# BICLab/Spike2Former

Measured on AMD Instinct MI355X. Metric: fwd+bwd images/sec, 512x512 T=4 ADE20K-150, higher is better.
Workload: dtype f32 (fp32-equivalent: bf16 hi+mid+lo split operands on bf16 MFMA, fp32 accumulate; spike maps stored as bf16, exact); 1 GPU; C2: 512x512 T=4 K=150 Meta-SpikeFormer [64, 128, 256, 360] + MaskFormer head, per-GPU batch 2; global_batch=2, parallelism=dp1, weights=random-init (name-seeded)

## Files before the change

include/s2f.h:

```cpp
#ifndef S2F_H
#define S2F_H

#include <stdint.h>

#ifdef __cplusplus
extern "C" {
#endif

#define S2F_OK 0
#define S2F_EINVAL (-1)
#define S2F_EALIGN (-2)
#define S2F_ELAUNCH (-3)

#define S2F_ABI_VERSION 36
#define S2F_STAT_SLOTS 256

int s2f_version(void);
const char* s2f_last_error(void);

void* s2f_event_create(void);
void s2f_event_destroy(void* event);
int s2f_time_next_call(void* start_event, void* stop_event);
int s2f_event_elapsed_us(void* start_event, void* stop_event, double* microseconds);

int64_t s2f_lif_mask_words(int64_t n);

int s2f_lif_fwd(const float* x, const float* v_in, void* y, float* v_out, uint64_t* mask, uint8_t* count_u8,
                uint64_t* stats, int64_t n, float vth, int D, int y_bf16, void* stream);

int s2f_lif_bwd(const float* gy, const float* gv_out, const uint64_t* mask, float* gx, int64_t n, float vth, int D,
                void* stream);
int s2f_lif_bwd_ports(const float* gy, const float* gy2, const float* gv_out, const uint64_t* mask, const float* skip, float* gx,
                      int64_t n, float vth, int D, void* stream);

int s2f_lif_leaky_fwd(const float* x, const float* v_in, void* y, float* v_out, uint64_t* mask, uint64_t* stats, int64_t n, float vth,
                      int D, float tau, int decay_input, int y_bf16, void* stream);
int s2f_lif_leaky_bwd(const float* gy, const float* gv_out, const uint64_t* mask, float* gx, float* gv_in, int64_t n, float vth, int D,
// ... 94 lines not shown
int s2f_spike_gemm_dw_pipe_ok(int batch, int M, int K, int L);
int s2f_spike_gemm_dw_pipe(const float* dY, const uint16_t* X, float* dW, int batch, int M, int K, int L, int accumulate, int cfg,
                           int target_wgs, void* stream);
int s2f_spike_gemm_dw_pipe_grouped(const int64_t* jobs, int njobs, int cfg, int target_wgs, void* stream);
int s2f_spike_conv3x3_dw_pipe_ok(int batch, int M, int C, int H, int W);
int s2f_shift1_bf16(const uint16_t* X, uint16_t* Xs, int64_t n, void* stream);
int s2f_spike_conv3x3_dw_pipe(const int64_t* jobs, int njobs, int cfg, int target_wgs, void* stream);

int s2f_gemm_bn_lif_fwd(const uint16_t* a_pack, const uint16_t* X, const float* conv_bias, const float* running_mean,
                        const float* running_var, const float* gamma, const float* beta, float eps, const float* residual,
                        float* u_out, const float* v_in, void* y_bf16, float* v_out, uint64_t* stats, int batch, int M, int N,
                        int K, float vth, int D, void* stream);
int s2f_conv3x3_bn_lif_fwd(const uint16_t* w_pack, const uint16_t* X, const float* conv_bias, const float* running_mean,
                           const float* running_var, const float* gamma, const float* beta, float eps, const float* residual,
                           float* u_out, const float* v_in, void* y_bf16, float* v_out, uint64_t* stats, int batch, int M, int C,
                           int H, int W, float vth, int D, void* stream);
int64_t s2f_pack_elems(int M, int K);
int s2f_pack_bf16x3(const float* src, uint16_t* dst, int M, int K, int mode, int C, void* stream);
int s2f_pack_bf16x3_multi(const int64_t* jobs, int njobs, int64_t total_workgroups, void* stream);
int s2f_pgemm_nn_bf16(const uint16_t* a_pack, const uint16_t* X, const float* bias, float* Y, int batch, int M, int N, int K,
                      int terms, int cfg, void* stream);
int s2f_pgemm_dx_f32(const uint16_t* w_pack, const float* G, int64_t g_batch_stride, float* DX, int64_t dx_batch_stride,
                     int batch, int Mo, int Ki, int N, float beta, int cfg, void* stream);
int s2f_dense_gemm_bn_lif_fwd(const uint16_t* const* w_packs, int groups, const float* X, int64_t x_batch_stride, int64_t x_group_stride,
                              const float* conv_bias, const float* running_mean, const float* running_var, const float* gamma,
                              const float* beta, float eps, const float* residual, float* u_out, void* y_bf16, uint64_t* stats,
                              int batch, int K, int M, int N, float vth, int D, void* stream);
int s2f_pgemm_dx_f32_grouped(const uint16_t* const* w_packs, int groups, const float* G, int64_t g_batch_stride,
                             int64_t g_group_stride, float* DX, int64_t dx_batch_stride, int64_t dx_group_stride, float* bn_partials,
                             int64_t partials_group_stride, int batch, int Mo, int Ki, int N, void* stream);
int s2f_pgemm_conv3x3_bf16(const uint16_t* w_pack, const uint16_t* X, const float* bias, float* Y, int batch, int M, int C, int H,
                           int W, int cfg, void* stream);
int s2f_pgemm_conv3x3_f32(const uint16_t* w_pack, const float* X, float* Y, int batch, int M, int C, int H, int W, int cfg,
                          void* stream);
int64_t s2f_bn_partials_count(int batch, int N);
int s2f_pgemm_nn_bf16_stats(const uint16_t* a_pack, const uint16_t* X, float* Y, float* bn_partials, int batch, int M, int N, int K,
                            void* stream);
int s2f_pgemm_conv3x3_bf16_stats(const uint16_t* w_pack, const uint16_t* X, float* Y, float* bn_partials, int batch, int M, int C,
                                 int H, int W, void* stream);
int s2f_pgemm_dx_f32_stats(const uint16_t* w_pack, const float* G, int64_t g_batch_stride, float* DX, int64_t dx_batch_stride,
                           float* bn_partials, int batch, int Mo, int Ki, int N, void* stream);
int s2f_bn_partials_finalize(const float* partials, int64_t P, const float* conv_bias, double* sums_out, int64_t N, int64_t C,
                             int64_t L, void* stream);
int s2f_bn_bwd_ports_ok(int64_t N, int64_t C, int64_t L, int training, int D);
int s2f_bn_act_bwd_ports(const float* z, const float* conv_bias, const float* stat, const float* gamma, const float* g_u,
                         const float* g_y, const float* g_y2, const float* g_v, const uint64_t* mask, double* sums_zeroed, float* gz,
// ... 136 lines not shown
```

spike2former_amd/_lib.py:

```python
import ctypes
import os

import torch

_HERE = os.path.dirname(os.path.abspath(__file__))
LIB_PATH = os.environ.get("S2F_LIB") or os.path.join(_HERE, "libs2f_hip.so")

_p, _i, _i64, _f = ctypes.c_void_p, ctypes.c_int, ctypes.c_int64, ctypes.c_float

SIGNATURES = {
    "s2f_version": (_i, []),
    "s2f_last_error": (ctypes.c_char_p, []),
    "s2f_event_create": (_p, []),
    "s2f_event_destroy": (None, [_p]),
    "s2f_time_next_call": (_i, [_p, _p]),
    "s2f_event_elapsed_us": (_i, [_p, _p, ctypes.POINTER(ctypes.c_double)]),
    "s2f_lif_mask_words": (_i64, [_i64]),
    "s2f_lif_fwd": (_i, [_p, _p, _p, _p, _p, _p, _p, _i64, _f, _i, _i, _p]),
    "s2f_lif_bwd": (_i, [_p, _p, _p, _p, _i64, _f, _i, _p]),
    "s2f_lif_bwd_ports": (_i, [_p] * 6 + [_i64, _f, _i, _p]),
    "s2f_lif_leaky_fwd": (_i, [_p, _p, _p, _p, _p, _p, _i64, _f, _i, _f, _i, _i, _p]),
    "s2f_lif_leaky_bwd": (_i, [_p, _p, _p, _p, _p, _i64, _f, _i, _f, _i, _p]),
    "s2f_sum2_lif_fwd": (_i, [_p] * 7 + [_i64] * 4 + [_f, _i, _i, _p]),
    "s2f_sum2_lif_bwd": (_i, [_p] * 5 + [_i64, _i, _p]),
# ... 43 lines not shown
    "s2f_split_gemm": (_i, [_p, _i64, _i64, _i, _p, _i64, _i, _i64, _i, _p, _i64, _f, _i, _i, _i, _i, _i, _i, _p]),
    "s2f_spike_gemm_dw": (_i, [_p, _p, _p, _i, _i, _i, _i, _i, _i, _p]),
    "s2f_to_bf16_exact": (_i, [_p, _p, _i64, _p]),
    "s2f_spike_gemm_fwd_bf16": (_i, [_p] * 4 + [_i] * 7 + [_p]),
    "s2f_spike_conv3x3_fwd_bf16": (_i, [_p, _p, _p, _p] + [_i] * 8 + [_p]),
    "s2f_spike_gemm_dw_bf16": (_i, [_p, _p, _p, _i, _i, _i, _i, _i, _p]),
    "s2f_spike_gemm_fwd_bf16_ex": (_i, [_p, _i64, _p, _i64, _i, _i64, _p, _i64, _f, _p, _i, _i, _i, _i, _i, _i, _p]),
    "s2f_pgemm_nn_bf16_ex": (_i, [_p, _i64, _p, _i64, _i, _i64, _p, _i64, _f, _p, _i, _i, _i, _i, _p]),
    "s2f_spike_gemm_dw_grouped": (_i, [_p, _i, _i, _p]),
    "s2f_spike_gemm_dw_pipe_ok": (_i, [_i] * 4),
    "s2f_spike_gemm_dw_pipe": (_i, [_p, _p, _p] + [_i] * 7 + [_p]),
    "s2f_spike_gemm_dw_pipe_grouped": (_i, [_p, _i, _i, _i, _p]),
    "s2f_spike_conv3x3_dw_pipe_ok": (_i, [_i] * 5),
    "s2f_shift1_bf16": (_i, [_p, _p, _i64, _p]),
    "s2f_spike_conv3x3_dw_pipe": (_i, [_p, _i, _i, _i, _p]),
    "s2f_spike_conv3x3_dw_bf16": (_i, [_p, _p, _p] + [_i] * 6 + [_p]),
    "s2f_gemm_bn_lif_fwd": (_i, [_p] * 7 + [_f] + [_p] * 6 + [_i] * 4 + [_f, _i, _p]),
    "s2f_conv3x3_bn_lif_fwd": (_i, [_p] * 7 + [_f] + [_p] * 6 + [_i] * 5 + [_f, _i, _p]),
    "s2f_pack_elems": (_i64, [_i, _i]),
    "s2f_pack_bf16x3_multi": (_i, [_p, _i, _i64, _p]),
    "s2f_pgemm_nn_bf16": (_i, [_p] * 4 + [_i] * 6 + [_p]),
    "s2f_pack_bf16x3": (_i, [_p, _p, _i, _i, _i, _i, _p]),
    "s2f_pgemm_dx_f32": (_i, [_p, _p, _i64, _p, _i64] + [_i] * 4 + [_f, _i, _p]),
    "s2f_gemm_dw_general": (_i, [_p, _i64, _p, _i64, _p] + [_i] * 5 + [_p]),
    "s2f_pgemm_conv3x3_bf16": (_i, [_p, _p, _p, _p] + [_i] * 6 + [_p]),
    "s2f_pgemm_conv3x3_f32": (_i, [_p, _p, _p] + [_i] * 6 + [_p]),
    "s2f_gemm_dw_general_grouped": (_i, [_p, _i, _p]),
    "s2f_bn_partials_count": (_i64, [_i, _i]),
    "s2f_pgemm_nn_bf16_stats": (_i, [_p] * 4 + [_i] * 4 + [_p]),
    "s2f_pgemm_conv3x3_bf16_stats": (_i, [_p] * 4 + [_i] * 5 + [_p]),
    "s2f_pgemm_dx_f32_grouped": (_i, [_p, _i, _p, _i64, _i64, _p, _i64, _i64, _p, _i64] + [_i] * 4 + [_p]),
    "s2f_dense_gemm_bn_lif_fwd": (_i, [_p, _i, _p, _i64, _i64, _p, _p, _p, _p, _p, _f, _p, _p, _p, _p, _i, _i, _i, _i, _f, _i, _p]),
    "s2f_pgemm_dx_f32_stats": (_i, [_p, _p, _i64, _p, _i64, _p] + [_i] * 4 + [_p]),
    "s2f_bn_partials_finalize": (_i, [_p, _i64, _p, _p, _i64, _i64, _i64, _p]),
    "s2f_bn_act_bwd_split": (_i, [_p] * 13 + [_i64] * 3 + [_i, _f, _i, _p]),
    "s2f_bn_act_bwd_ports": (_i, [_p] * 14 + [_i64] * 3 + [_i, _f, _i, _p]),
    "s2f_bn_bwd_ports_ok": (_i, [_i64, _i64, _i64, _i, _i]),
    "s2f_mask_cost_bins": (_i, [_p, _p, _p, _i, _i, _i64, _i, _f, _f, _f, _p]),
    "s2f_mask_loss_seg_partials": (_i64, [_i] * 4),
    "s2f_mask_loss_seg_fwd": (_i, [_p] * 5 + [_i] * 4 + [_f, _f, _p]),
    "s2f_mask_loss_seg_bwd": (_i, [_p] * 5 + [_i] * 4 + [_f, _f, _p]),
    "s2f_lsa_tables": (_i, [_p] * 6 + [_i] * 4 + [_p]),
    "s2f_lsa_tables_ex": (_i, [_p] * 6 + [_i] * 5 + [_p]),
    "s2f_spike_gemm_dw_bf16_split": (_i, [_p, _i64, _p, _p] + [_i] * 5 + [_p]),
    "s2f_spike_gemm_dw_grouped_split": (_i, [_p, _i, _i, _p]),
    "s2f_pgemm_dx_split": (_i, [_p, _p, _i64, _p] + [_i] * 5 + [_p]),
# ... 54 lines not shown
```

spike2former_amd/csrc/pgemm.hip:

```cpp
#include "gemm_common.h"
#include <cstdlib>
#include <type_traits>

#pragma clang fp contract(fast)

namespace {

constexpr int PK = 32;
constexpr int PR = 64;
constexpr int PTERM = PR * PK;
constexpr int PBLOCK = 3 * PTERM;

typedef __attribute__((address_space(3))) void lds_void;
typedef const __attribute__((address_space(1))) void gbl_void;

__device__ __forceinline__ void dma16(const void* src, void* lds_dst) {
  __builtin_amdgcn_global_load_lds((gbl_void*)src, (lds_void*)lds_dst, 16, 0, 0);
}
template <int OFF>
__device__ __forceinline__ s16x4 lds_tr16_asm(unsigned byte_addr) {
  s16x4 r;
  asm volatile("ds_read_b64_tr_b16 %0, %1 offset:%2" : "=v"(r) : "v"(byte_addr), "n"(OFF));
  return r;
}
// ... 397 lines not shown
      const int row = m0 + wm * (32 * MI) + i * 32 + (r & 3) + 8 * (r >> 2) + 4 * (lane >> 5);
      bv[r] = bias ? bias[min(row, M - 1)] : 0.f;
    }
#pragma unroll
    for (int j = 0; j < NJ; ++j) {
      const int col = n0 + (wn * NJ + j) * 32 + (lane & 31);
#pragma unroll
      for (int r = 0; r < 16; ++r) {
        const int row = m0 + wm * (32 * MI) + i * 32 + (r & 3) + 8 * (r >> 2) + 4 * (lane >> 5);
        if (row < M && col < N) Yb[(int64_t)row * N + col] = EX ? (acc[i][j][r] + bv[r]) * ex.out_scale : acc[i][j][r] + bv[r];
      }
    }
  }
  if constexpr (STATS)
    epi_row_partials<MI, NJ, WMW, WNW>(acc, part, n_tiles * (int)gridDim.y, reinterpret_cast<float*>(smem), m0, n0, M, N,
                                       b * n_tiles + nt, wm, wn, lane, (int)threadIdx.x);
}

struct TnGroups {
  const unsigned short* wp[4];
  int64_t g_stride, dx_stride, part_stride;
};

template <int MI, int NJ, int WMW, int WNW, int EPI, int KS = 1, bool STATS = false, bool GROUPED = false>
__global__ __launch_bounds__(64 * WMW * WNW) void pg_tn_f32_kernel(const unsigned short* __restrict__ Wp,
                                                                  const float* __restrict__ G, float* __restrict__ DX, int Mo,
                                                                  int Ki, int N, int KbW, int n_tiles, int m_tiles, float beta,
                                                                  int64_t g_batch_stride, int64_t dx_batch_stride,
                                                                  float* __restrict__ part = nullptr, TnGroups grp = TnGroups{},
                                                                  BnLifEpi ep = BnLifEpi{}) {
  if constexpr (GROUPED) {
    static_assert(EPI == 0 || EPI == 3, "grouped form: plain store or the eval-mode BatchNorm epilogue");
    const int g = blockIdx.z;
    Wp = grp.wp[g];
    G += g * grp.g_stride;
    if (EPI == 0) DX += g * grp.dx_stride;
    if (STATS) part += g * grp.part_stride;
    if constexpr (EPI == 3) {
      if (ep.conv_bias) ep.conv_bias += g * Ki;
      ep.mean += g * Ki, ep.var += g * Ki, ep.gamma += g * Ki, ep.beta += g * Ki;
      if (ep.residual) ep.residual += g * grp.dx_stride;
      if (ep.u_out) ep.u_out += g * grp.dx_stride;
      if (ep.y) ep.y += g * grp.dx_stride;
    }
  }
  constexpr bool BETA = EPI == 1;
  constexpr int BM = 32 * MI * WMW, BN = 32 * NJ * WNW, NW = WMW * WNW, T = 64 * NW;
  constexpr int KC = 16 * KS;
  constexpr int A_SLICE = 3 * (BM / 32) * 1024;
  constexpr int A_BYTES = KS * A_SLICE, B_TERM = KC * BN * 2, B_BYTES = 3 * B_TERM, STAGE = A_BYTES + B_BYTES;
  constexpr int NA = 3 * (BM / 32);
  constexpr int NQ = KC * BN / 4 / T;
  static_assert(NQ >= 1 && (KC * BN / 4) % T == 0, "tile too small for the thread count");
  __shared__ __attribute__((aligned(1024))) unsigned char smem[2 * STAGE];

  const int tiles = n_tiles * m_tiles;
  int pid = blockIdx.x;
  if (tiles % 8 == 0) pid = (pid % 8) * (tiles / 8) + pid / 8;
  const int mt = pid % m_tiles, nt = pid / m_tiles;
  const int b = blockIdx.y;
  const int m0 = mt * BM, n0 = nt * BN;
  const float* Gb = G + (int64_t)b * g_batch_stride;
  float* Db = DX + (int64_t)b * dx_batch_stride;
  const int tid = threadIdx.x, lane = tid & 63;
  const int wave = __builtin_amdgcn_readfirstlane((int)(tid >> 6));
  const int wm = wave / WNW, wn = wave % WNW;
  const int nk_all = (Mo + KC - 1) / KC;
  const int per_z = (nk_all + (int)gridDim.z - 1) / (int)gridDim.z;
  const int t_first = EPI == 2 ? (int)blockIdx.z * per_z : 0;
  const int nk = EPI == 2 ? max(0, min(nk_all - t_first, per_z)) : nk_all;
  if (EPI == 2 && nk == 0) return;

  auto issue_a = [&](int tl, int st) __attribute__((always_inline)) {
    unsigned char* sb = smem + st * STAGE;
#pragma unroll
    for (int ks = 0; ks < KS; ++ks) {
      const int c0 = (t_first + tl) * KC + 16 * ks;
      const unsigned short* rows = Wp + (int64_t)(c0 / PR) * KbW * PBLOCK + (c0 % PR) * PK + lane * 8;
#pragma unroll
      for (int q = 0; q < (NA + NW - 1) / NW; ++q) {
        const int idx = wave + q * NW;
        if (NA % NW != 0 && idx >= NA) break;
        const int term = idx / (BM / 32), p = idx % (BM / 32);
        const int kb = min(m0 / PK + p, KbW - 1);
// ... 20 lines not shown
      const int k = p / (BN / 4), c4 = p % (BN / 4);
      const int off = k * BN + ((((c4 >> 3) ^ (k & 3)) << 5) | ((c4 & 7) << 2));
      unsigned int h0, m0_, l0_, h1, m1, l1;
      s2f_split3x2(breg[q].x, breg[q].y, h0, m0_, l0_);
      s2f_split3x2(breg[q].z, breg[q].w, h1, m1, l1);
      *reinterpret_cast<u32x2*>(Bs + off) = u32x2{h0, h1};
      *reinterpret_cast<u32x2*>(Bs + KC * BN + off) = u32x2{m0_, m1};
      *reinterpret_cast<u32x2*>(Bs + 2 * KC * BN + off) = u32x2{l0_, l1};
    }
  };

  f32x16 acc[MI][NJ];
#pragma unroll
  for (int i = 0; i < MI; ++i)
#pragma unroll
    for (int j = 0; j < NJ; ++j)
#pragma unroll
      for (int r = 0; r < 16; ++r) acc[i][j][r] = 0.f;

  const int kl = (lane & 15) >> 2, piece = lane & 3, hcol = (lane >> 4) & 1, kh = lane >> 5;
  int boff[NJ];
#pragma unroll
  for (int j = 0; j < NJ; ++j) boff[j] = (8 * kh + kl) * BN + (((wn * NJ + j) ^ kl) << 5) + 16 * hcol + 4 * piece;
  int aoff[MI][2];
#pragma unroll
  for (int i = 0; i < MI; ++i)
#pragma unroll
    for (int half = 0; half < 2; ++half) {
      const int row = 8 * kh + kl + 4 * half;
      const int c = (2 * hcol + (piece >> 1)) ^ ((2 * kh + half) & 3);
      aoff[i][half] = (wm * MI + i) * 512 + row * 32 + c * 8 + 4 * (piece & 1);
    }

  const unsigned smem_a = lds_addr(smem);
  auto compute = [&](int st) __attribute__((always_inline)) {
    union BF {
      bf16x8 v;
      s16x4 h[2];
    } bfrag[3][NJ], afrag[3][MI];
    const unsigned sb0 = smem_a + st * STAGE;
#pragma unroll
    for (int ks = 0; ks < KS; ++ks) {
      const unsigned sb = sb0 + ks * A_SLICE;
      const unsigned sbb = sb0 + ks * (16 * BN * 2);
#pragma unroll
      for (int j = 0; j < NJ; ++j) {
        const unsigned a = sbb + boff[j] * 2;
        bfrag[0][j].h[0] = lds_tr16_asm<A_BYTES>(a);
        bfrag[0][j].h[1] = lds_tr16_asm<A_BYTES + 4 * BN * 2>(a);
        bfrag[1][j].h[0] = lds_tr16_asm<A_BYTES + B_TERM>(a);
        bfrag[1][j].h[1] = lds_tr16_asm<A_BYTES + B_TERM + 4 * BN * 2>(a);
        bfrag[2][j].h[0] = lds_tr16_asm<A_BYTES + 2 * B_TERM>(a);
        bfrag[2][j].h[1] = lds_tr16_asm<A_BYTES + 2 * B_TERM + 4 * BN * 2>(a);
      }
#pragma unroll
      for (int i = 0; i < MI; ++i) {
        afrag[0][i].h[0] = lds_tr16_asm<0>(sb + aoff[i][0] * 2);
        afrag[0][i].h[1] = lds_tr16_asm<0>(sb + aoff[i][1] * 2);
      }
#pragma unroll
      for (int i = 0; i < MI; ++i) {
        afrag[1][i].h[0] = lds_tr16_asm<(BM / 32) * 1024>(sb + aoff[i][0] * 2);
        afrag[1][i].h[1] = lds_tr16_asm<(BM / 32) * 1024>(sb + aoff[i][1] * 2);
      }
#pragma unroll
      for (int i = 0; i < MI; ++i) {
        afrag[2][i].h[0] = lds_tr16_asm<2 * (BM / 32) * 1024>(sb + aoff[i][0] * 2);
        afrag[2][i].h[1] = lds_tr16_asm<2 * (BM / 32) * 1024>(sb + aoff[i][1] * 2);
      }
#pragma unroll
      for (int ta = 0; ta < 3; ++ta) {
        if (ta == 0) lds_wait<4 * MI>();
        if (ta == 1) lds_wait<2 * MI>();
        if (ta == 2) lds_wait<0>();
#pragma unroll
        for (int i = 0; i < MI; ++i)
#pragma unroll
          for (int tb = 0; tb < 3; ++tb)
            if (ta + tb < 3)
#pragma unroll
              for (int j = 0; j < NJ; ++j)
                mfma_bf16(acc[i][j], afrag[ta][i].v, bfrag[tb][j].v);
      }
    }
  };

  fetch_b(0);
  issue_a(0, 0);
  stage_b(0);
  if (nk > 1) fetch_b(1);
  for (int t = 0; t < nk; ++t) {
    const int st = t & 1;
    if (t + 1 < nk)
      wait_vm_and_barrier<NQ>();
    else
      wait_vm_and_barrier<0>();
    if (t + 1 < nk) {
      stage_b(st ^ 1);
      issue_a(t + 1, st ^ 1);
      if (t + 2 < nk) fetch_b(t + 2);
    }
    compute(st);
  }

  mfma_fence(acc);
  if constexpr (EPI == 3) {
    static_assert(2 * STAGE >= BM * BN * 4, "the output tile must fit the stages it is transposed through");
    epi_bn_lif<MI, NJ, WMW, WNW>(acc, ep, smem, m0, n0, Ki, N, b, wm, wn, lane, wave, dx_batch_stride);
    return;
  }
#pragma unroll
  for (int i = 0; i < MI; ++i)
#pragma unroll
    for (int j = 0; j < NJ; ++j) {
      const int col = n0 + (wn * NJ + j) * 32 + (lane & 31);
      float prev[16];
      if (BETA) {
#pragma unroll
        for (int r = 0; r < 16; ++r) {
          const int row = m0 + (wm * MI + i) * 32 + (r & 3) + 8 * (r >> 2) + 4 * (lane >> 5);
          prev[r] = Db[(int64_t)min(row, Ki - 1) * N + min(col, N - 1)];
        }
      }
#pragma unroll
      for (int r = 0; r < 16; ++r) {
        const int row = m0 + (wm * MI + i) * 32 + (r & 3) + 8 * (r >> 2) + 4 * (lane >> 5);
        if (row < Ki && col < N) {
          if (EPI == 2)
            atomicAdd(Db + (int64_t)row * N + col, acc[i][j][r]);
          else
            Db[(int64_t)row * N + col] = BETA ? acc[i][j][r] + beta * prev[r] : acc[i][j][r];
        }
      }
    }
  if constexpr (EPI == 0 && STATS)
    epi_row_partials<MI, NJ, WMW, WNW>(acc, part, n_tiles * (int)gridDim.y, reinterpret_cast<float*>(smem), m0, n0, Ki, N,
                                       b * n_tiles + nt, wm, wn, lane, tid);
}

template <int MI, int NJ, int WMW, int WNW, int NST>
__global__ __launch_bounds__(64 * WMW * WNW) void pg_tn_split_kernel(const unsigned short* __restrict__ Wp,
                                                                    const unsigned short* __restrict__ Gs, int64_t plane_stride,
                                                                    float* __restrict__ DX, int Mo, int Ki, int N, int KbW,
                                                                    int n_tiles, int m_tiles) {
  constexpr int BM = 32 * MI * WMW, BN = 32 * NJ * WNW, NW = WMW * WNW;
  constexpr int KC = 16;
  constexpr int A_BYTES = 3 * (BM / 32) * 1024, B_TERM = KC * BN * 2, B_BYTES = 3 * B_TERM, STAGE = A_BYTES + B_BYTES;
  constexpr int NA = 3 * (BM / 32), NAW = (NA + NW - 1) / NW;
  constexpr int NBT = B_TERM / 1024, NB = 3 * NBT, NBW = NB / NW;
  static_assert(NB % NW == 0 && BN == 128, "tile shape");
  constexpr int LPW = NAW + NBW;
  __shared__ __attribute__((aligned(1024))) unsigned char smem[NST * STAGE];

  const int tiles = n_tiles * m_tiles;
  int pid = blockIdx.x;
  if (tiles % 8 == 0) pid = (pid % 8) * (tiles / 8) + pid / 8;
  const int mt = pid % m_tiles, nt = pid / m_tiles;
// ... 460 lines not shown
constexpr bool conv_g2_built(int cfg) {
  for (const ConvForm& f : kConvForms)
    if (f.g == 2 && (f.cfgs >> cfg & 1)) return true;
  return false;
}

constexpr PgTile kTnSplitTiles[] = {
    {1, 2, 2, 2, 2, 3},
    {2, 1, 2, 2, 2, 3},
    {3, 2, 2, 2, 2, 2},
    {4, 1, 2, 2, 2, 2},
};

constexpr PgTile kTnTiles[] = {
    {1, 2, 2, 2, 2, 1},
    {2, 1, 2, 2, 2, 1},
    {3, 1, 2, 4, 2, 1},
    {4, 1, 1, 2, 4, 1},
    {5, 1, 1, 1, 4, 1},
    {7, 1, 1, 2, 4, 2},
    {8, 1, 2, 2, 2, 2},
    {9, 1, 2, 4, 2, 2},
    {10, 1, 1, 2, 4, 4},
};
struct TnForm {
  int epi;
  bool stats, grouped;
  unsigned cfgs;
};
constexpr TnForm kTnForms[] = {
    {2, false, false, cfg_set(1, 2, 3, 4, 5)},
    {1, false, false, cfg_set(1, 2, 3, 4, 5)},
    {0, true, false, cfg_set(1, 2, 3, 4, 5, 7, 8, 9, 10)},
    {0, false, false, cfg_set(1, 2, 3, 4, 5, 7, 8, 9, 10)},
    {0, true, true, cfg_set(3, 5, 7)},
    {0, false, true, cfg_set(3, 5, 7)},
    {3, false, true, cfg_set(5, 7, 9, 10)},
};

bool launch_pg_nn(int cfg, int terms, int epi, bool ex_form, hipStream_t s, const uint16_t* a_pack, const uint16_t* X, const float* bias,
                  float* Y, int batch, int M, int N, int K, int64_t xbs, const BnLifEpi& ep, float* part, const NnEx& ex) {
  const int Kb = (K + PK - 1) / PK, n_tiles = (N + 127) / 128;
  bool ok = false;
  s2f_dispatch<kNnForms>(
      [&](const NnForm& e) { return e.terms == terms && e.epi == epi && e.stats == (part != nullptr) && e.ex == ex_form; }, [&](auto f) {
        constexpr NnForm F = kNnForms[f];
        ok = s2f_dispatch<kNnTiles>([&](const PgTile& e) { return e.cfg == cfg && (F.cfgs >> e.cfg & 1); }, [&](auto i) {
          constexpr PgTile T = kNnTiles[i];
          if constexpr (F.cfgs >> T.cfg & 1) {
            const int m_tiles = (M + T.rows() - 1) / T.rows();
            S2F_LAUNCH(true, true, (pg_nn_kernel<T.MI, T.NJ, T.WMW, T.WNW, F.terms, T.extra, F.epi, F.stats, F.ex>),
                       dim3(n_tiles * m_tiles, batch), dim3(T.threads()), 0, s, a_pack, X, bias, Y, M, N, K, Kb, n_tiles, m_tiles, xbs,
                       ep, part, ex);
          }
        });
      });
  return ok;
}

template <class TwoSteps>
bool launch_pg_conv(int cfg, bool conv, int bt, int epi, const TwoSteps& two_steps, hipStream_t s, const uint16_t* a_pack, const void* X,
                    const float* bias, float* Y, int batch, int M, int N, int K, int Kb, Conv3 geo, float* part, const BnLifEpi& ep) {
  const int n_tiles = (N + 127) / 128;
  bool ok = false;
  s2f_dispatch<kConvTiles>([&](const PgTile& e) { return e.cfg == cfg && (e.extra != 0) == conv; }, [&](auto i) {
    constexpr PgTile T = kConvTiles[i];
    const int m_tiles = (M + T.rows() - 1) / T.rows();
    const bool stats = part != nullptr && bt == 1;
    const int g = (conv_g2_built(T.cfg) && two_steps((int64_t)n_tiles * m_tiles * batch)) ? 2 : 1;
    ok = s2f_dispatch<kConvForms>(
        [&](const ConvForm& e) { return e.bt == bt && e.epi == epi && e.stats == stats && e.g == g && (e.cfgs >> T.cfg & 1); }, [&](auto f) {
          constexpr ConvForm F = kConvForms[f];
          if constexpr (F.cfgs >> T.cfg & 1)
            S2F_LAUNCH(true, true, (pg_conv_kernel<T.MI, T.NJ, T.WMW, T.WNW, F.bt, T.extra != 0, F.stats, F.epi, F.g>),
                       dim3(n_tiles * m_tiles, batch), dim3(T.threads()), 0, s, a_pack, X, bias, Y, M, N, K, Kb, n_tiles, m_tiles, geo,
                       part, ep);
        });
  });
  return ok;
}

bool launch_pg_tn(int cfg, int epi, bool grouped, hipStream_t s, const uint16_t* w_pack, const float* G, float* DX, int batch, int zdim,
                  int Mo, int Ki, int N, float beta, int64_t g_batch_stride, int64_t dx_batch_stride, float* part, const TnGroups& grp,
                  const BnLifEpi& ep) {
  const int KbW = (Ki + PK - 1) / PK, n_tiles = (N + 127) / 128;
  bool ok = false;
  s2f_dispatch<kTnForms>([&](const TnForm& e) { return e.epi == epi && e.stats == (part != nullptr) && e.grouped == grouped; }, [&](auto f) {
    constexpr TnForm F = kTnForms[f];
    ok = s2f_dispatch<kTnTiles>([&](const PgTile& e) { return e.cfg == cfg && (F.cfgs >> e.cfg & 1); }, [&](auto i) {
      constexpr PgTile T = kTnTiles[i];
      if constexpr (F.cfgs >> T.cfg & 1) {
        const int m_tiles = (Ki + T.rows() - 1) / T.rows();
        S2F_LAUNCH(true, true, (pg_tn_f32_kernel<T.MI, T.NJ, T.WMW, T.WNW, F.epi, T.extra, F.stats, F.grouped>),
                   dim3(n_tiles * m_tiles, batch, zdim), dim3(T.threads()), 0, s, w_pack, G, DX, Mo, Ki, N, KbW, n_tiles, m_tiles, beta,
                   g_batch_stride, dx_batch_stride, part, grp, ep);
      }
    });
  });
  return ok;
}

}

extern "C" int64_t s2f_pack_elems(int M, int K) { return (int64_t)((M + PR - 1) / PR) * ((K + PK - 1) / PK) * PBLOCK; }

extern "C" int s2f_pack_bf16x3_multi(const int64_t* jobs, int njobs, int64_t total_workgroups, void* stream) {
  if (njobs == 0) return S2F_OK;
  S2F_REQUIRE(jobs && njobs > 0 && total_workgroups > 0 && total_workgroups < (1ll << 31), S2F_EINVAL,
              "s2f_pack_bf16x3_multi: bad job table");
  hipLaunchKernelGGL(pack_multi_kernel, dim3((unsigned)total_workgroups), dim3(256), 0, (hipStream_t)stream,
                     reinterpret_cast<const long long*>(jobs), njobs);
  return s2f_check_launch("s2f_pack_bf16x3_multi");
}

static int pgemm_nn_impl(const uint16_t* a_pack, const uint16_t* X, const float* bias, float* Y, int batch, int M, int N, int K,
                         int terms, int cfg, float* part, void* stream) {
  S2F_REQUIRE(a_pack && X && Y, S2F_EINVAL, "s2f_pgemm_nn_bf16: null pointer");
  S2F_REQUIRE(!part || (!bias && (reinterpret_cast<uintptr_t>(part) & 7u) == 0), S2F_EINVAL,
// ... 153 lines not shown
  return conv_launch("s2f_pgemm_conv3x3_bf16", w_pack, X, false, bias, Y, batch, M, C, H, W, cfg, stream);
}

extern "C" int s2f_pgemm_conv3x3_bf16_stats(const uint16_t* w_pack, const uint16_t* X, float* Y, float* bn_partials, int batch,
                                            int M, int C, int H, int W, void* stream) {
  S2F_REQUIRE(bn_partials, S2F_EINVAL, "s2f_pgemm_conv3x3_bf16_stats: null partials");
  return conv_launch("s2f_pgemm_conv3x3_bf16_stats", w_pack, X, false, nullptr, Y, batch, M, C, H, W, 0, stream, bn_partials);
}

extern "C" int s2f_pgemm_conv3x3_f32(const uint16_t* w_pack, const float* X, float* Y, int batch, int M, int C, int H, int W,
                                     int cfg, void* stream) {
  return conv_launch("s2f_pgemm_conv3x3_f32", w_pack, X, true, nullptr, Y, batch, M, C, H, W, cfg, stream);
}

extern "C" int s2f_pack_bf16x3(const float* src, uint16_t* dst, int M, int K, int mode, int C, void* stream) {
  S2F_REQUIRE(src && dst && M > 0 && K > 0 && mode >= 0 && mode <= 3, S2F_EINVAL, "s2f_pack_bf16x3: bad arguments");
  S2F_REQUIRE((mode != 1 && mode != 2) || C > 0, S2F_EINVAL, "s2f_pack_bf16x3: conv modes need C");
  const int64_t wgs = (int64_t)((M + PR - 1) / PR) * ((K + PK - 1) / PK) * (PTERM / 1024);
  hipLaunchKernelGGL(pack_one_kernel, dim3((unsigned)wgs), dim3(256), 0, (hipStream_t)stream, src, dst, M, K, mode, C);
  return s2f_check_launch("s2f_pack_bf16x3");
}

static int pgemm_dx_impl(const uint16_t* w_pack, const float* G, int64_t g_batch_stride, float* DX, int64_t dx_batch_stride,
                         int batch, int Mo, int Ki, int N, float beta, int cfg, float* part, void* stream) {
  if (g_batch_stride == 0) g_batch_stride = (int64_t)Mo * N;
  S2F_REQUIRE(!part || (beta == 0.f && (reinterpret_cast<uintptr_t>(part) & 7u) == 0), S2F_EINVAL,
              "s2f_pgemm_dx_f32_stats: plain-store form only; partials 8-byte aligned");
  if (dx_batch_stride == 0) dx_batch_stride = (int64_t)Ki * N;
  S2F_REQUIRE((g_batch_stride & 3) == 0 && (dx_batch_stride & 3) == 0, S2F_EALIGN, "s2f_pgemm_dx_f32: batch strides must keep 16-byte alignment");
  S2F_REQUIRE(w_pack && G && DX, S2F_EINVAL, "s2f_pgemm_dx_f32: null pointer");
  S2F_REQUIRE(batch > 0 && batch < 65536 && Mo > 0 && Ki > 0 && N >= 4 && (N & 3) == 0, S2F_EINVAL,
              "s2f_pgemm_dx_f32: bad sizes (N=%d must be a positive multiple of 4)", N);
  S2F_REQUIRE(s2f_aligned16(w_pack) && s2f_aligned16(G) && s2f_aligned16(DX), S2F_EALIGN,
              "s2f_pgemm_dx_f32: pointers must be 16-byte aligned");
  hipStream_t s = (hipStream_t)stream;
  const int n_tiles = (N + 127) / 128;
  static const char* force = getenv("S2F_PG_DX_CFG");
  int c = cfg > 0 ? cfg : (force ? atoi(force) : 0);
  static const char* t3e = getenv("S2F_PG_DX_T3");
  const int64_t t3 = t3e ? atoll(t3e) : 192;
  if (c <= 0) c = Ki <= 32 ? 5 : (Ki > 64 && (int64_t)n_tiles * batch * ((Ki + 127) / 128) >= t3) ? 3 : (beta == 0.f ? 7 : 4);
  static const char* ks4 = getenv("S2F_PG_DX_KS4");
  if (c == 7 && !(ks4 && ks4[0] == '0') && Mo >= 128 && (int64_t)n_tiles * batch * ((Ki + 63) / 64) <= 512) c = 10;
  int zsplit = 1;
  {
    const int64_t wgs = (int64_t)n_tiles * batch * ((Ki + 63) / 64);
    const int steps = (Mo + 15) / 16;
    while ((beta == 0.f || beta == 1.f) && !part && wgs * zsplit < 128 && steps / (zsplit * 2) >= 16) zsplit *= 2;
  }
  if (zsplit > 1) {
    S2F_REQUIRE(dx_batch_stride == (int64_t)Ki * N, S2F_EINVAL, "s2f_pgemm_dx_f32: the split form needs a dense DX");
    if (beta == 0.f && s2f_zero_async(DX, sizeof(float) * (size_t)batch * Ki * N, s) != S2F_OK)
      return s2f_check_launch("s2f_pgemm_dx_f32 zero");
    c = 4;
  }
  S2F_REQUIRE(c < 7 || c > 10 || (zsplit == 1 && beta == 0.f), S2F_EINVAL, "s2f_pgemm_dx_f32: cfg %d is the plain store form", c);
  const bool ok = launch_pg_tn(c, zsplit > 1 ? 2 : beta != 0.f ? 1 : 0, false, s, w_pack, G, DX, batch, zsplit, Mo, Ki, N, beta,
                               g_batch_stride, dx_batch_stride, part, TnGroups{}, BnLifEpi{});
  S2F_REQUIRE(ok, S2F_EINVAL, "s2f_pgemm_dx_f32: unknown cfg %d", c);
  return s2f_check_launch("s2f_pgemm_dx_f32");
}

extern "C" int s2f_pgemm_dx_f32(const uint16_t* w_pack, const float* G, int64_t g_batch_stride, float* DX,
                                int64_t dx_batch_stride, int batch, int Mo, int Ki, int N, float beta, int cfg, void* stream) {
  return pgemm_dx_impl(w_pack, G, g_batch_stride, DX, dx_batch_stride, batch, Mo, Ki, N, beta, cfg, nullptr, stream);
}

extern "C" int s2f_pgemm_dx_f32_stats(const uint16_t* w_pack, const float* G, int64_t g_batch_stride, float* DX,
                                      int64_t dx_batch_stride, float* bn_partials, int batch, int Mo, int Ki, int N,
                                      void* stream) {
  S2F_REQUIRE(bn_partials, S2F_EINVAL, "s2f_pgemm_dx_f32_stats: null partials");
  return pgemm_dx_impl(w_pack, G, g_batch_stride, DX, dx_batch_stride, batch, Mo, Ki, N, 0.f, 0, bn_partials, stream);
}

extern "C" int s2f_dense_gemm_bn_lif_fwd(const uint16_t* const* w_packs, int groups, const float* X, int64_t x_batch_stride,
                                         int64_t x_group_stride, const float* conv_bias, const float* running_mean,
                                         const float* running_var, const float* gamma, const float* beta, float eps,
                                         const float* residual, float* u_out, void* y_bf16, uint64_t* stats, int batch, int K,
                                         int M, int N, float vth, int D, void* stream) {
  S2F_REQUIRE(w_packs && X && running_mean && running_var && gamma && beta && groups >= 1 && groups <= 4, S2F_EINVAL,
              "s2f_dense_gemm_bn_lif_fwd: null pointer / 1..4 groups");
  S2F_REQUIRE(u_out || y_bf16, S2F_EINVAL, "s2f_dense_gemm_bn_lif_fwd: neither u_out nor y requested");
  S2F_REQUIRE(batch > 0 && batch < 65536 && M > 0 && K > 0 && N >= 4 && (N & 3) == 0, S2F_EINVAL,
// ... 51 lines not shown
```

spike2former_amd/ops/gemm.py:

```python
import torch

from .config import cfg
from .core import *
from .misc import channel_sum, transpose_last2




def bmm_small(a, b, reduce_batch=False):
    _need_cuda(a, b)
    B, M, K = a.shape
    N = b.shape[2]
    if b.shape[0] != B or b.shape[1] != K:
        raise RuntimeError(f"bmm_small: {tuple(a.shape)} @ {tuple(b.shape)}")
    c = torch.empty((M, N) if reduce_batch else (B, M, N), dtype=torch.float32, device=a.device)
    if c.numel() == 0:
        return c
    if K == 0 or B == 0:
        return c.zero_()
    check(lib.s2f_bmm_f32(_ptr(a), a.stride(0), a.stride(1), a.stride(2), _ptr(b), b.stride(0), b.stride(1), b.stride(2), _ptr(c),
                          0 if reduce_batch else M * N, N, 1, B, M, N, K, int(bool(reduce_batch)), _stream()), "s2f_bmm_f32")
    return c


# ... 615 lines not shown
                for t in range(T):
                    for b in range(B):
                        check(lib.s2f_spike_gemm_dw(_ptr(g[b]), _ptr(mf[t, b]), _ptr(ge[t, b]), 1, Q, C, HW, 1, 3, _stream()),
                              "s2f_spike_gemm_dw")
            else:
                ge = torch.stack([bmm_small(g, mf[t].transpose(1, 2)) for t in range(T)], 0)
            ge.mul_(ctx.scale)
        if ctx.needs_input_grad[1]:
            gmf = torch.empty_like(mf)
            if ctx.mfma:
                et = e.permute(0, 1, 3, 2).reshape(T * B * C, Q)
                a_split, Rpad, Kpad = _split_rows(et, 128)
                for t in range(T):
                    check(lib.s2f_split_gemm(_ptr(a_split) + 2 * t * B * C * Kpad, C * Kpad, Rpad * Kpad, 1, _ptr(g), Q * HW, Q,
                                             0, 3, _ptr(gmf[t]), C * HW, ctx.scale, B, C, HW, Q, (C + 127) // 128 * 128, Kpad,
                                             _stream()), "s2f_split_gemm")
            else:
                es = e * ctx.scale
                for t in range(T):
                    gmf[t].copy_(bmm_small(es[t].transpose(1, 2), g))
        return ge, gmf, None, None


def mask_einsum(e, mf, scale, e_exact=False):
    return _MaskEinsum.apply(e, mf, float(scale), bool(e_exact))


class _MaskEinsumFolded(torch.autograd.Function):

    @staticmethod
    def forward(ctx, e, sdata, stok, W, bias, scale, T, B, e_exact):
        _need_cuda(e, W, bias, spikes=sdata)
        Q, Co = e.shape[2], e.shape[3]
        C, HW = sdata.shape[1], sdata.shape[2]
        e = e.contiguous()
        sdata = sdata.contiguous()
        dev = e.device
        ew = _mm_tm(e.reshape(-1, Co), transpose_last2(W.detach().unsqueeze(0))[0]).view(T, B, Q, C)
        acat = ew.permute(1, 2, 0, 3).reshape(B, Q, T * C).contiguous()
        rowb = None
        if bias is not None:
            rowb = (e.sum(0) * bias.view(1, 1, -1)).sum(-1).contiguous()
        out = torch.empty(B, Q, HW, dtype=torch.float32, device=dev)
        if HW % 8 == 0 and C % 32 == 0:
            pe = int(lib.s2f_pack_elems(Q, T * C))
            a_pack = torch.empty(B, pe, dtype=torch.int16, device=dev)
# ... 7 lines not shown
            Kpad = T * C
            a_split = torch.empty(B, 3, Mpad, Kpad, dtype=torch.int16, device=dev)
            for b in range(B):
                check(lib.s2f_split_bf16x3(_ptr(acat[b]), _ptr(a_split[b]), Q, T * C, Mpad, Kpad, _stream()), "s2f_split_bf16x3")
            _time_next("spike_gemm_fwd", 4 * B * HW * (T * C + Q), 2 * B * Q * HW * T * C, moved=B * HW * (2 * T * C + 4 * Q))
            check(lib.s2f_spike_gemm_fwd_bf16_ex(_ptr(a_split), 3 * Mpad * Kpad, _ptr(sdata), C * HW, C, B * C * HW, _ptr(rowb),
                                                 Q if rowb is not None else 0, scale, _ptr(out), B, Q, HW, T * C, Mpad, Kpad, _stream()),
                  "s2f_spike_gemm_fwd_bf16_ex")
        ctx.save_for_backward(e, sdata, W, bias, ew)
        ctx.cfg = (scale, T, B)
        return out

    @staticmethod
    def backward(ctx, g):
        e, sdata, W, bias, ew = ctx.saved_tensors
        scale, T, B = ctx.cfg
        Q, Co = e.shape[2], e.shape[3]
        C, HW = sdata.shape[1], sdata.shape[2]
        g = g.contiguous()
        dev = g.device
        gs = ge = gW = gb = None
        S = sdata.view(T, B, C, HW)
        if (ctx.needs_input_grad[1] or ctx.needs_input_grad[2]) and HW % 4 == 0:
            ews = ew * scale
            gs = torch.empty(T * B, C, HW, dtype=torch.float32, device=dev)
            _time_next("dx_gemm", 4 * T * B * HW * (C + Q), 2 * T * B * Q * HW * C)
            for t in range(T):
                for b in range(B):
                    _mtm_tm(ews[t, b], g[b], out=gs[t * B + b])
        elif ctx.needs_input_grad[1] or ctx.needs_input_grad[2]:
            G = torch.empty(T, B, Co, HW, dtype=torch.float32, device=dev)
            es = e * scale
            for t in range(T):
                G[t].copy_(bmm_small(es[t].transpose(1, 2), g))
            gs = dx_gemm(W, G.view(T * B, Co, HW))
        if ctx.needs_input_grad[0] or ctx.needs_input_grad[3] or ctx.needs_input_grad[4]:
            H = torch.empty(T, B, Q, C, dtype=torch.float32, device=dev)
            xb = sdata.dtype == torch.bfloat16
            _time_next("spike_gemm_dw", 4 * T * B * HW * (C + Q), 2 * T * B * Q * HW * C, moved=T * B * HW * ((2 if xb else 4) * C + 4 * Q))
            if xb and T * B <= 56 and HW % 4 == 0:
                import ctypes
                H.zero_()
                flat = []
                for t in range(T):
                    for b in range(B):
                        flat += [g[b].data_ptr(), S[t, b].data_ptr(), H[t, b].data_ptr(), 1, Q, C, HW]
                arr = (ctypes.c_int64 * len(flat))(*flat)
                if (cfg.DW_PIPE and lib.s2f_spike_gemm_dw_pipe_ok(1, Q, C, HW) and g.data_ptr() % 16 == 0 and S.data_ptr() % 16 == 0
                        and (Q * HW) % 4 == 0 and (C * HW) % 8 == 0):
                    check(lib.s2f_spike_gemm_dw_pipe_grouped(arr, T * B, 0, 0, _stream()), "s2f_spike_gemm_dw_pipe_grouped")
                else:
                    check(lib.s2f_spike_gemm_dw_grouped(arr, T * B, 64, _stream()), "s2f_spike_gemm_dw_grouped")
# ... 46 lines not shown
```

Before: 56.41 images/s.

## Batch mask-einsum input gradient into one stacked row-block dx GEMM launch

```diff
diff --git a/include/s2f.h b/include/s2f.h
--- a/include/s2f.h
+++ b/include/s2f.h
@@ -12,7 +12,7 @@
 #define S2F_EALIGN (-2)
 #define S2F_ELAUNCH (-3)
 
-#define S2F_ABI_VERSION 36
+#define S2F_ABI_VERSION 37
 #define S2F_STAT_SLOTS 256
 
 int s2f_version(void);
@@ -153,6 +153,9 @@
                       int terms, int cfg, void* stream);
 int s2f_pgemm_dx_f32(const uint16_t* w_pack, const float* G, int64_t g_batch_stride, float* DX, int64_t dx_batch_stride,
                      int batch, int Mo, int Ki, int N, float beta, int cfg, void* stream);
+int s2f_pgemm_dx_f32_rowblocks(const uint16_t* w_pack, int64_t w_batch_stride, const float* G, int64_t g_batch_stride, float* DX,
+                               int64_t dx_batch_stride, int rows_per_block, int64_t block_stride, int batch, int Mo, int Ki, int N,
+                               int cfg, void* stream);
 int s2f_dense_gemm_bn_lif_fwd(const uint16_t* const* w_packs, int groups, const float* X, int64_t x_batch_stride, int64_t x_group_stride,
                               const float* conv_bias, const float* running_mean, const float* running_var, const float* gamma,
                               const float* beta, float eps, const float* residual, float* u_out, void* y_bf16, uint64_t* stats,
diff --git a/spike2former_amd/_lib.py b/spike2former_amd/_lib.py
--- a/spike2former_amd/_lib.py
+++ b/spike2former_amd/_lib.py
@@ -89,6 +89,7 @@
     "s2f_pgemm_nn_bf16": (_i, [_p] * 4 + [_i] * 6 + [_p]),
     "s2f_pack_bf16x3": (_i, [_p, _p, _i, _i, _i, _i, _p]),
     "s2f_pgemm_dx_f32": (_i, [_p, _p, _i64, _p, _i64] + [_i] * 4 + [_f, _i, _p]),
+    "s2f_pgemm_dx_f32_rowblocks": (_i, [_p, _i64, _p, _i64, _p, _i64, _i, _i64] + [_i] * 5 + [_p]),
     "s2f_gemm_dw_general": (_i, [_p, _i64, _p, _i64, _p] + [_i] * 5 + [_p]),
     "s2f_pgemm_conv3x3_bf16": (_i, [_p, _p, _p, _p] + [_i] * 6 + [_p]),
     "s2f_pgemm_conv3x3_f32": (_i, [_p, _p, _p] + [_i] * 6 + [_p]),
diff --git a/spike2former_amd/csrc/pgemm.hip b/spike2former_amd/csrc/pgemm.hip
--- a/spike2former_amd/csrc/pgemm.hip
+++ b/spike2former_amd/csrc/pgemm.hip
@@ -443,13 +443,15 @@
   int64_t g_stride, dx_stride, part_stride;
 };
 
-template <int MI, int NJ, int WMW, int WNW, int EPI, int KS = 1, bool STATS = false, bool GROUPED = false>
-__global__ __launch_bounds__(64 * WMW * WNW) void pg_tn_f32_kernel(const unsigned short* __restrict__ Wp,
+template <int MI, int NJ, int WMW, int WNW, int EPI, int KS = 1, bool STATS = false, bool GROUPED = false, bool ROWBLK = false>
+__global__ __launch_bounds__(64 * WMW * WNW, (MI * WMW == 8 ? 4 : 1)) void pg_tn_f32_kernel(const unsigned short* __restrict__ Wp,
                                                                   const float* __restrict__ G, float* __restrict__ DX, int Mo,
                                                                   int Ki, int N, int KbW, int n_tiles, int m_tiles, float beta,
                                                                   int64_t g_batch_stride, int64_t dx_batch_stride,
                                                                   float* __restrict__ part = nullptr, TnGroups grp = TnGroups{},
-                                                                  BnLifEpi ep = BnLifEpi{}) {
+                                                                  BnLifEpi ep = BnLifEpi{}, int rows_per_block = 0,
+                                                                  int64_t block_stride = 0, int64_t w_batch_stride = 0) {
+  static_assert(!ROWBLK || (EPI == 0 && !STATS && !GROUPED), "row blocks: the plain-store form only");
   if constexpr (GROUPED) {
     static_assert(EPI == 0 || EPI == 3, "grouped form: plain store or the eval-mode BatchNorm epilogue");
     const int g = blockIdx.z;
@@ -481,6 +483,7 @@
   const int mt = pid % m_tiles, nt = pid / m_tiles;
   const int b = blockIdx.y;
   const int m0 = mt * BM, n0 = nt * BN;
+  if constexpr (ROWBLK) Wp += (int64_t)b * w_batch_stride;
   const float* Gb = G + (int64_t)b * g_batch_stride;
   float* Db = DX + (int64_t)b * dx_batch_stride;
   const int tid = threadIdx.x, lane = tid & 63;
@@ -547,15 +550,13 @@
   int boff[NJ];
 #pragma unroll
   for (int j = 0; j < NJ; ++j) boff[j] = (8 * kh + kl) * BN + (((wn * NJ + j) ^ kl) << 5) + 16 * hcol + 4 * piece;
-  int aoff[MI][2];
-#pragma unroll
-  for (int i = 0; i < MI; ++i)
-#pragma unroll
-    for (int half = 0; half < 2; ++half) {
-      const int row = 8 * kh + kl + 4 * half;
-      const int c = (2 * hcol + (piece >> 1)) ^ ((2 * kh + half) & 3);
-      aoff[i][half] = (wm * MI + i) * 512 + row * 32 + c * 8 + 4 * (piece & 1);
-    }
+  int aoff[2];
+#pragma unroll
+  for (int half = 0; half < 2; ++half) {
+    const int row = 8 * kh + kl + 4 * half;
+    const int c = (2 * hcol + (piece >> 1)) ^ ((2 * kh + half) & 3);
+    aoff[half] = wm * MI * 512 + row * 32 + c * 8 + 4 * (piece & 1);
+  }
 
   const unsigned smem_a = lds_addr(smem);
   auto compute = [&](int st) __attribute__((always_inline)) {
@@ -578,20 +579,26 @@
         bfrag[2][j].h[0] = lds_tr16_asm<A_BYTES + 2 * B_TERM>(a);
         bfrag[2][j].h[1] = lds_tr16_asm<A_BYTES + 2 * B_TERM + 4 * BN * 2>(a);
       }
-#pragma unroll
-      for (int i = 0; i < MI; ++i) {
-        afrag[0][i].h[0] = lds_tr16_asm<0>(sb + aoff[i][0] * 2);
-        afrag[0][i].h[1] = lds_tr16_asm<0>(sb + aoff[i][1] * 2);
-      }
-#pragma unroll
-      for (int i = 0; i < MI; ++i) {
-        afrag[1][i].h[0] = lds_tr16_asm<(BM / 32) * 1024>(sb + aoff[i][0] * 2);
-        afrag[1][i].h[1] = lds_tr16_asm<(BM / 32) * 1024>(sb + aoff[i][1] * 2);
-      }
-#pragma unroll
-      for (int i = 0; i < MI; ++i) {
-        afrag[2][i].h[0] = lds_tr16_asm<2 * (BM / 32) * 1024>(sb + aoff[i][0] * 2);
-        afrag[2][i].h[1] = lds_tr16_asm<2 * (BM / 32) * 1024>(sb + aoff[i][1] * 2);
+      static_assert(MI <= 2, "the row blocks of a wavefront are written out below");
+      const unsigned a0 = sb + aoff[0] * 2, a1 = sb + aoff[1] * 2;
+      constexpr int AT = (BM / 32) * 1024;
+      afrag[0][0].h[0] = lds_tr16_asm<0>(a0);
+      afrag[0][0].h[1] = lds_tr16_asm<0>(a1);
+      if constexpr (MI == 2) {
+        afrag[0][MI - 1].h[0] = lds_tr16_asm<1024>(a0);
+        afrag[0][MI - 1].h[1] = lds_tr16_asm<1024>(a1);
+      }
+      afrag[1][0].h[0] = lds_tr16_asm<AT>(a0);
+      afrag[1][0].h[1] = lds_tr16_asm<AT>(a1);
+      if constexpr (MI == 2) {
+        afrag[1][MI - 1].h[0] = lds_tr16_asm<AT + 1024>(a0);
+        afrag[1][MI - 1].h[1] = lds_tr16_asm<AT + 1024>(a1);
+      }
+      afrag[2][0].h[0] = lds_tr16_asm<2 * AT>(a0);
+      afrag[2][0].h[1] = lds_tr16_asm<2 * AT>(a1);
+      if constexpr (MI == 2) {
+        afrag[2][MI - 1].h[0] = lds_tr16_asm<2 * AT + 1024>(a0);
+        afrag[2][MI - 1].h[1] = lds_tr16_asm<2 * AT + 1024>(a1);
       }
 #pragma unroll
       for (int ta = 0; ta < 3; ++ta) {
@@ -635,7 +642,16 @@
     return;
   }
 #pragma unroll
-  for (int i = 0; i < MI; ++i)
+  for (int i = 0; i < MI; ++i) {
+    [[maybe_unused]] int64_t roff[ROWBLK ? 16 : 1];
+    if constexpr (ROWBLK) {
+#pragma unroll
+      for (int r = 0; r < 16; ++r) {
+        const int row = m0 + (wm * MI + i) * 32 + (r & 3) + 8 * (r >> 2) + 4 * (lane >> 5);
+        const int blk = row / rows_per_block;
+        roff[r] = blk * block_stride + (int64_t)(row - blk * rows_per_block) * N;
+      }
+    }
 #pragma unroll
     for (int j = 0; j < NJ; ++j) {
       const int col = n0 + (wn * NJ + j) * 32 + (lane & 31);
@@ -653,11 +669,14 @@
         if (row < Ki && col < N) {
           if (EPI == 2)
             atomicAdd(Db + (int64_t)row * N + col, acc[i][j][r]);
+          else if constexpr (ROWBLK)
+            Db[roff[r] + col] = acc[i][j][r];
           else
             Db[(int64_t)row * N + col] = BETA ? acc[i][j][r] + beta * prev[r] : acc[i][j][r];
         }
       }
     }
+  }
   if constexpr (EPI == 0 && STATS)
     epi_row_partials<MI, NJ, WMW, WNW>(acc, part, n_tiles * (int)gridDim.y, reinterpret_cast<float*>(smem), m0, n0, Ki, N,
                                        b * n_tiles + nt, wm, wn, lane, tid);
@@ -1164,20 +1183,22 @@
     {8, 1, 2, 2, 2, 2},
     {9, 1, 2, 4, 2, 2},
     {10, 1, 1, 2, 4, 4},
+    {11, 2, 2, 4, 2, 1},
 };
 struct TnForm {
   int epi;
-  bool stats, grouped;
+  bool stats, grouped, rowblk;
   unsigned cfgs;
 };
 constexpr TnForm kTnForms[] = {
-    {2, false, false, cfg_set(1, 2, 3, 4, 5)},
-    {1, false, false, cfg_set(1, 2, 3, 4, 5)},
-    {0, true, false, cfg_set(1, 2, 3, 4, 5, 7, 8, 9, 10)},
-    {0, false, false, cfg_set(1, 2, 3, 4, 5, 7, 8, 9, 10)},
-    {0, true, true, cfg_set(3, 5, 7)},
-    {0, false, true, cfg_set(3, 5, 7)},
-    {3, false, true, cfg_set(5, 7, 9, 10)},
+    {2, false, false, false, cfg_set(1, 2, 3, 4, 5)},
+    {1, false, false, false, cfg_set(1, 2, 3, 4, 5, 11)},
+    {0, true, false, false, cfg_set(1, 2, 3, 4, 5, 7, 8, 9, 10)},
+    {0, false, false, false, cfg_set(1, 2, 3, 4, 5, 7, 8, 9, 10, 11)},
+    {0, true, true, false, cfg_set(3, 5, 7)},
+    {0, false, true, false, cfg_set(3, 5, 7)},
+    {3, false, true, false, cfg_set(5, 7, 9, 10)},
+    {0, false, false, true, cfg_set(3, 5, 7, 11)},
 };
 
 bool launch_pg_nn(int cfg, int terms, int epi, bool ex_form, hipStream_t s, const uint16_t* a_pack, const uint16_t* X, const float* bias,
@@ -1224,18 +1245,19 @@
 
 bool launch_pg_tn(int cfg, int epi, bool grouped, hipStream_t s, const uint16_t* w_pack, const float* G, float* DX, int batch, int zdim,
                   int Mo, int Ki, int N, float beta, int64_t g_batch_stride, int64_t dx_batch_stride, float* part, const TnGroups& grp,
-                  const BnLifEpi& ep) {
+                  const BnLifEpi& ep, int rows_per_block = 0, int64_t block_stride = 0, int64_t w_batch_stride = 0) {
   const int KbW = (Ki + PK - 1) / PK, n_tiles = (N + 127) / 128;
   bool ok = false;
-  s2f_dispatch<kTnForms>([&](const TnForm& e) { return e.epi == epi && e.stats == (part != nullptr) && e.grouped == grouped; }, [&](auto f) {
+  const bool rowblk = rows_per_block > 0;
+  s2f_dispatch<kTnForms>([&](const TnForm& e) { return e.epi == epi && e.stats == (part != nullptr) && e.grouped == grouped && e.rowblk == rowblk; }, [&](auto f) {
     constexpr TnForm F = kTnForms[f];
     ok = s2f_dispatch<kTnTiles>([&](const PgTile& e) { return e.cfg == cfg && (F.cfgs >> e.cfg & 1); }, [&](auto i) {
       constexpr PgTile T = kTnTiles[i];
       if constexpr (F.cfgs >> T.cfg & 1) {
         const int m_tiles = (Ki + T.rows() - 1) / T.rows();
-        S2F_LAUNCH(true, true, (pg_tn_f32_kernel<T.MI, T.NJ, T.WMW, T.WNW, F.epi, T.extra, F.stats, F.grouped>),
+        S2F_LAUNCH(true, true, (pg_tn_f32_kernel<T.MI, T.NJ, T.WMW, T.WNW, F.epi, T.extra, F.stats, F.grouped, F.rowblk>),
                    dim3(n_tiles * m_tiles, batch, zdim), dim3(T.threads()), 0, s, w_pack, G, DX, Mo, Ki, N, KbW, n_tiles, m_tiles, beta,
-                   g_batch_stride, dx_batch_stride, part, grp, ep);
+                   g_batch_stride, dx_batch_stride, part, grp, ep, rows_per_block, block_stride, w_batch_stride);
       }
     });
   });
@@ -1435,7 +1457,9 @@
 }
 
 static int pgemm_dx_impl(const uint16_t* w_pack, const float* G, int64_t g_batch_stride, float* DX, int64_t dx_batch_stride,
-                         int batch, int Mo, int Ki, int N, float beta, int cfg, float* part, void* stream) {
+                         int batch, int Mo, int Ki, int N, float beta, int cfg, float* part, void* stream, int rows_per_block = 0,
+                         int64_t block_stride = 0, int64_t w_batch_stride = 0) {
+  const bool rowblk = rows_per_block > 0;
   if (g_batch_stride == 0) g_batch_stride = (int64_t)Mo * N;
   S2F_REQUIRE(!part || (beta == 0.f && (reinterpret_cast<uintptr_t>(part) & 7u) == 0), S2F_EINVAL,
               "s2f_pgemm_dx_f32_stats: plain-store form only; partials 8-byte aligned");
@@ -1454,12 +1478,12 @@
   const int64_t t3 = t3e ? atoll(t3e) : 192;
   if (c <= 0) c = Ki <= 32 ? 5 : (Ki > 64 && (int64_t)n_tiles * batch * ((Ki + 127) / 128) >= t3) ? 3 : (beta == 0.f ? 7 : 4);
   static const char* ks4 = getenv("S2F_PG_DX_KS4");
-  if (c == 7 && !(ks4 && ks4[0] == '0') && Mo >= 128 && (int64_t)n_tiles * batch * ((Ki + 63) / 64) <= 512) c = 10;
+  if (c == 7 && !rowblk && !(ks4 && ks4[0] == '0') && Mo >= 128 && (int64_t)n_tiles * batch * ((Ki + 63) / 64) <= 512) c = 10;
   int zsplit = 1;
   {
     const int64_t wgs = (int64_t)n_tiles * batch * ((Ki + 63) / 64);
     const int steps = (Mo + 15) / 16;
-    while ((beta == 0.f || beta == 1.f) && !part && wgs * zsplit < 128 && steps / (zsplit * 2) >= 16) zsplit *= 2;
+    while ((beta == 0.f || beta == 1.f) && !part && !rowblk && c != 11 && wgs * zsplit < 128 && steps / (zsplit * 2) >= 16) zsplit *= 2;
   }
   if (zsplit > 1) {
     S2F_REQUIRE(dx_batch_stride == (int64_t)Ki * N, S2F_EINVAL, "s2f_pgemm_dx_f32: the split form needs a dense DX");
@@ -1469,9 +1493,23 @@
   }
   S2F_REQUIRE(c < 7 || c > 10 || (zsplit == 1 && beta == 0.f), S2F_EINVAL, "s2f_pgemm_dx_f32: cfg %d is the plain store form", c);
   const bool ok = launch_pg_tn(c, zsplit > 1 ? 2 : beta != 0.f ? 1 : 0, false, s, w_pack, G, DX, batch, zsplit, Mo, Ki, N, beta,
-                               g_batch_stride, dx_batch_stride, part, TnGroups{}, BnLifEpi{});
+                               g_batch_stride, dx_batch_stride, part, TnGroups{}, BnLifEpi{}, rows_per_block, block_stride, w_batch_stride);
   S2F_REQUIRE(ok, S2F_EINVAL, "s2f_pgemm_dx_f32: unknown cfg %d", c);
   return s2f_check_launch("s2f_pgemm_dx_f32");
+}
+
+extern "C" int s2f_pgemm_dx_f32_rowblocks(const uint16_t* w_pack, int64_t w_batch_stride, const float* G, int64_t g_batch_stride,
+                                          float* DX, int64_t dx_batch_stride, int rows_per_block, int64_t block_stride, int batch,
+                                          int Mo, int Ki, int N, int cfg, void* stream) {
+  S2F_REQUIRE(rows_per_block > 0 && block_stride >= 0 && (block_stride & 3) == 0, S2F_EINVAL,
+              "s2f_pgemm_dx_f32_rowblocks: rows_per_block > 0 and block_stride %% 4 == 0 needed");
+  S2F_REQUIRE(w_batch_stride >= 0 && (w_batch_stride & 7) == 0, S2F_EALIGN,
+              "s2f_pgemm_dx_f32_rowblocks: the packs of the batch elements must keep 16-byte alignment");
+  S2F_REQUIRE(Ki <= rows_per_block || block_stride >= (int64_t)rows_per_block * N, S2F_EINVAL,
+              "s2f_pgemm_dx_f32_rowblocks: the row blocks overlap (block_stride < rows_per_block * N)");
+  S2F_REQUIRE(dx_batch_stride != 0, S2F_EINVAL, "s2f_pgemm_dx_f32_rowblocks: dx_batch_stride must be given");
+  return pgemm_dx_impl(w_pack, G, g_batch_stride, DX, dx_batch_stride, batch, Mo, Ki, N, 0.f, cfg, nullptr, stream, rows_per_block,
+                       block_stride, w_batch_stride);
 }
 
 extern "C" int s2f_pgemm_dx_f32(const uint16_t* w_pack, const float* G, int64_t g_batch_stride, float* DX,
diff --git a/spike2former_amd/ops/gemm.py b/spike2former_amd/ops/gemm.py
--- a/spike2former_amd/ops/gemm.py
+++ b/spike2former_amd/ops/gemm.py
@@ -661,6 +661,33 @@
         return ge, gmf, None, None
 
 
+def _mask_ds_stacked(ew, g, scale):
+    T, B, Q, C = ew.shape
+    HW = g.shape[-1]
+    gs = torch.empty(T * B, C, HW, dtype=torch.float32, device=g.device)
+    acat_s = (ew * scale).permute(1, 2, 0, 3).reshape(B, Q, T * C).contiguous()
+    pe = int(lib.s2f_pack_elems(Q, T * C))
+    a_pack = torch.empty(B, pe, dtype=torch.int16, device=g.device)
+    for b in range(B):
+        check(lib.s2f_pack_bf16x3(_ptr(acat_s[b]), _ptr(a_pack[b]), Q, T * C, 0, 0, _stream()), "s2f_pack_bf16x3")
+    _time_next("dx_gemm", 4 * T * B * HW * (C + Q), 2 * T * B * Q * HW * C)
+    check(lib.s2f_pgemm_dx_f32_rowblocks(_ptr(a_pack), pe, _ptr(g), Q * HW, _ptr(gs), C * HW, C, B * C * HW, B, Q, T * C, HW, 0,
+                                         _stream()), "s2f_pgemm_dx_f32_rowblocks")
+    return gs
+
+
+def _mask_ds_per_slice(ew, g, scale):
+    T, B, Q, C = ew.shape
+    HW = g.shape[-1]
+    ews = ew * scale
+    gs = torch.empty(T * B, C, HW, dtype=torch.float32, device=g.device)
+    _time_next("dx_gemm", 4 * T * B * HW * (C + Q), 2 * T * B * Q * HW * C)
+    for t in range(T):
+        for b in range(B):
+            _mtm_tm(ews[t, b], g[b], out=gs[t * B + b])
+    return gs
+
+
 def mask_einsum(e, mf, scale, e_exact=False):
     return _MaskEinsum.apply(e, mf, float(scale), bool(e_exact))
 
@@ -714,12 +741,7 @@
         gs = ge = gW = gb = None
         S = sdata.view(T, B, C, HW)
         if (ctx.needs_input_grad[1] or ctx.needs_input_grad[2]) and HW % 4 == 0:
-            ews = ew * scale
-            gs = torch.empty(T * B, C, HW, dtype=torch.float32, device=dev)
-            _time_next("dx_gemm", 4 * T * B * HW * (C + Q), 2 * T * B * Q * HW * C)
-            for t in range(T):
-                for b in range(B):
-                    _mtm_tm(ews[t, b], g[b], out=gs[t * B + b])
+            gs = _mask_ds_stacked(ew, g, scale)
         elif ctx.needs_input_grad[1] or ctx.needs_input_grad[2]:
             G = torch.empty(T, B, Co, HW, dtype=torch.float32, device=dev)
             es = e * scale
```

Result: no change. 56.51 images/s (median of 5 runs) (+0.2%).
